# CliMA/ClimaSeaIce.jl

Hardware: AMD Instinct MI355X
Metric: EVP sub-cycle cell-updates/s (higher is better)
Workload: dtype f64; 1 GPU; evp_subcycle_fplane_periodic_2048x2048_as_1x1_tiles_of_2048x2048_120substeps; substeps=120, mode=fast, halo=4, halo_exchange=none (one tile)

## Files before the change

climaseaice.jl_amd/_lib.py:

```python
import ctypes as C
import os

_HERE = os.path.dirname(os.path.abspath(__file__))
LIB_PATH = os.environ.get("CSI_HIP_LIBRARY", os.path.join(_HERE, "libcsi_hip.so"))

OK = 0
PERIODIC, BOUNDED, FULLY_CONNECTED, LEFT_CONNECTED, RIGHT_CONNECTED, RIGHT_FOLDED, LEFT_CONNECTED_RIGHT_FOLDED = 0, 1, 2, 3, 4, 5, 6
METRIC_UNIFORM, METRIC_PER_J, METRIC_FULL = 0, 1, 2
FIELD_IDS = ["U", "V", "H", "A", "S11", "S22", "S12", "UN", "VN", "P", "ALPHA", "DELTA", "ZETA_F", "ZETA_C",
             "GH", "GA", "HM", "AM", "UM", "VM", "TOP_U", "TOP_V", "BOT_U", "BOT_V", "MASS_FLUX",
             "HS", "GHS", "HSM", "MASS_FLUX_SNOW", "SNOWFALL_INTERCEPTED", "TU", "TUS", "FORCING_U", "FORCING_V", "GU", "GV"]
THERMO_FIELD_IDS = ["TOP_HEAT_FLUX", "BOTTOM_HEAT_FLUX", "SNOWFALL"]
F = {n: k for k, n in enumerate(FIELD_IDS + THERMO_FIELD_IDS)}
STRESS_NONE, STRESS_CONST, STRESS_FIELD, STRESS_SEMI_IMPLICIT = 0, 1, 2, 3
VEL_ZERO, VEL_CONST, VEL_FIELD = 0, 1, 2
STRESS_TOP, STRESS_BOTTOM = 0, 1
MODE_STRICT, MODE_FAST = 0, 1
PRESSURE_REPLACEMENT, PRESSURE_ICE_STRENGTH = 0, 1
RHEOLOGY_EVP, RHEOLOGY_VISCOUS = 0, 1
SOLVER_SPLIT_EXPLICIT, SOLVER_EXPLICIT = 0, 1
FLUX_CONSTANT, FLUX_ARRAY, FLUX_RADIATIVE_EMISSION = 0, 1, 2
HEAT_TOP, HEAT_BOTTOM = 0, 1
MAX_HEAT_FLUX_TERMS = 8

SYMBOLS = ["csi_version", "csi_context_create", "csi_context_destroy", "csi_last_error", "csi_sync", "csi_set_mode",
           "csi_grid_set", "csi_mask_set", "csi_field_bind", "csi_evp_params_set", "csi_stress_set",
           "csi_evp_initialize", "csi_evp_subcycle", "csi_evp_finalize", "csi_time_step_momentum",
           "csi_compute_tracer_tendencies", "csi_dynamic_step_tracers", "csi_cache_current_fields",
           "csi_update_state", "csi_fill_halo_local", "csi_time_step_fe", "csi_time_step_rk3",
           "csi_slab_thermo_step", "csi_slab_params_set", "csi_layered_thermo_step", "csi_snow_params_set", "csi_tile_set", "csi_comm_unique_id", "csi_comm_init", "csi_comm_count", "csi_local_group_create", "csi_local_group_destroy", "csi_comm_init_local", "csi_comm_init_host", "csi_halo_exchange",
           "csi_plan_exchange", "csi_set_fusion", "csi_set_exchange_interval", "csi_set_halo_transport", "csi_halo_transport", "csi_set_peer_tier", "csi_peer_tier", "csi_plan_ranges", "csi_profile_substeps", "csi_last_path", "csi_last_subcycle_ms", "csi_launches_per_substep", "csi_last_launches", "csi_plan_pair", "csi_plan_peer_chunks", "csi_free_drift_set", "csi_coriolis_rows_set", "csi_velocity_bc_set",
           "csi_immersed_flux_bc_set", "csi_coriolis_points_set", "csi_validate_all", "csi_debug_peer_abort", "csi_set_weno_weight_dtype", "csi_weno_weight_dtype", "csi_subcycle_stats_begin", "csi_subcycle_stats_end",
           "csi_set_tile_skipping", "csi_tile_activity", "csi_set_row_constant", "csi_row_constant_rows",
           "csi_rheology_set", "csi_momentum_solver_set", "csi_compute_momentum_tendencies",
           "csi_heat_fluxes_set", "csi_surface_solve_set"]


class Metrics(C.Structure):
    _fields_ = [("dx", C.c_double), ("dy", C.c_double),
                ("dxc", C.POINTER(C.c_double)), ("dxf", C.POINTER(C.c_double)),
                ("azc", C.POINTER(C.c_double)), ("azf", C.POINTER(C.c_double)),
                ("full", C.POINTER(C.c_double) * 12), ("full_ld", C.c_int64)]


class EvpParams(C.Structure):
    _fields_ = [("ice_compressive_strength", C.c_double), ("ice_compaction_hardening", C.c_double),
                ("yield_curve_eccentricity", C.c_double), ("minimum_plastic_stress", C.c_double),
                ("min_relaxation_parameter", C.c_double), ("max_relaxation_parameter", C.c_double),
# ... 74 lines not shown
        "csi_snow_params_set": [vp, C.POINTER(SnowParams)],
        "csi_tile_set": [vp, i32, i32, i32, i32, i32, i32],
        "csi_comm_unique_id": [C.POINTER(C.c_uint8)],
        "csi_comm_init": [vp, i32, i32, C.POINTER(C.c_uint8)],
        "csi_comm_count": [vp, C.POINTER(i32)],
        "csi_local_group_create": [i32, C.POINTER(vp)], "csi_comm_init_local": [vp, vp, i32],
        "csi_comm_init_host": [vp, C.c_char_p, i32, i32],
        "csi_halo_exchange": [vp, C.POINTER(i32), i32, i32],
        "csi_plan_ranges": [i32, i32, i32, i32, i32, i32, i32, C.POINTER(i32)],
        "csi_plan_pair": [i32, i32, i32, i32, i32, i32, i32, i32, C.POINTER(i32)],
        "csi_plan_peer_chunks": [i32, i32, i32, i32, i32, i32, i32, C.POINTER(i32), C.POINTER(i32), i32],
        "csi_set_exchange_interval": [vp, i32],
        "csi_set_halo_transport": [vp, i32], "csi_halo_transport": [vp, C.POINTER(i32)],
        "csi_set_peer_tier": [vp, i32], "csi_peer_tier": [vp, C.POINTER(i32)],
        "csi_set_fusion": [vp, i32], "csi_free_drift_set": [vp, i32],
        "csi_set_tile_skipping": [vp, i32], "csi_tile_activity": [vp, C.POINTER(i32), C.POINTER(i32), C.POINTER(i32)],
        "csi_set_row_constant": [vp, i32, dbl], "csi_row_constant_rows": [vp, C.POINTER(i32)],
        "csi_coriolis_rows_set": [vp, C.POINTER(C.c_double), C.POINTER(C.c_double), i32],
        "csi_velocity_bc_set": [vp, i32, i32, i32, dbl],
        "csi_coriolis_points_set": [vp, C.POINTER(C.c_double), C.POINTER(C.c_double), i64],
        "csi_immersed_flux_bc_set": [vp, i32, dbl, dbl, dbl, dbl],
        "csi_plan_exchange": [i32] * 14 + [C.POINTER(i32)],
        "csi_profile_substeps": [vp, dbl, i32, C.POINTER(dbl)],
        "csi_last_path": [vp, C.POINTER(i32), C.POINTER(i32), C.POINTER(i32)],
        "csi_last_subcycle_ms": [vp, C.POINTER(dbl)], "csi_launches_per_substep": [vp, C.POINTER(i32)],
        "csi_last_launches": [vp, C.POINTER(i32), C.POINTER(i32)],
        "csi_validate_all": [vp], "csi_debug_peer_abort": [vp], "csi_set_weno_weight_dtype": [vp, i32], "csi_weno_weight_dtype": [vp, C.POINTER(i32)], "csi_subcycle_stats_begin": [vp],
        "csi_subcycle_stats_end": [vp, C.POINTER(dbl), C.POINTER(i32), C.POINTER(i32)],
        "csi_rheology_set": [vp, i32, dbl], "csi_momentum_solver_set": [vp, i32], "csi_compute_momentum_tendencies": [vp, dbl],
        "csi_heat_fluxes_set": [vp, i32, C.POINTER(HeatFluxTerm), i32], "csi_surface_solve_set": [vp, C.POINTER(SurfaceSolve)],
# ... 22 lines not shown


def plan_pair(Nx, Ny, Hx, Hy, topo_x, topo_y, k=1, m=0):
    L = load()
    out = (C.c_int32 * 32)()
    rc = L.csi_plan_pair(Nx, Ny, Hx, Hy, topo_x, topo_y, k, m, out)
    if rc != OK:
        raise CsiError(rc, "csi_plan_pair")
    if not out[0]:
        return None
    r = lambda q: tuple(out[4 + 4 * q: 8 + 4 * q])
    return dict(nstrips=out[1], nchunks=out[2], rows=out[3], first_compute=r(0), second_compute=r(1), store_sigma=r(2),
                store_first_u=r(3), store_first_v=r(4), store_second=r(5), walls=bool(out[28]))


def plan_peer_chunks(Nx, Ny, Hx, Hy, peer_south=True, peer_north=True):
    out = (C.c_int32 * 8)()
    rows = (C.c_int32 * 4096)()
    rc = load().csi_plan_peer_chunks(Nx, Ny, Hx, Hy, int(peer_south), int(peer_north), 256, out, rows, 2048)
    if rc != OK:
        raise CsiError(rc, "csi_plan_peer_chunks")
    if not out[0]:
        return None
    n = out[2]
    return dict(nstrips=out[1], nchunks=n, rows=out[3], elo=out[4], ehi=out[5], nS=out[6], nN=out[7],
                chunks=[(rows[2 * q], rows[2 * q + 1]) for q in range(min(n, 2048))])


def plan_exchange(Nx, Ny, Hx, Hy, topo_x, topo_y, rx, ry, Rx, Ry, periodic_x, periodic_y, width, halo):
    out = (C.c_int32 * 40)()
# ... 101 lines not shown
```

climaseaice.jl_amd/csrc/csi_abi.hip:

```cpp
#include "csi_ctx.h"


static SlabDev slab_dev(const csi_slab_params* p) {
    SlabDev S{};
    S.k = p->conductivity; S.rho_bulk = p->sea_ice_density; S.rho_pure = p->density; S.rho_l = p->liquid_density;
    S.c_l = p->liquid_heat_capacity; S.c_i = p->heat_capacity; S.L0 = p->reference_latent_heat; S.T0 = p->reference_temperature;
    S.liq_slope = p->liquidus_slope; S.liq_T0 = p->freshwater_melting_temperature; S.S = p->bottom_salinity;
    S.hc = p->ice_consolidation_thickness; S.Tu = p->top_temperature; S.Qu = p->top_heat_flux; S.Qb = p->bottom_heat_flux;
    S.top_flux_kind = p->top_flux_kind; S.bot_flux_kind = p->bottom_flux_kind;
    S.top_bc_kind = p->top_bc_kind; S.ice_salinity = p->ice_salinity;
    return S;
}
static SnowDev snow_dev(const csi_snow_params* p) {
    SnowDev W{};
    W.k = p->conductivity; W.rho = p->snow_density; W.snowfall = p->snowfall; W.Tu = p->top_temperature; W.top_bc_kind = p->top_bc_kind;
    return W;
}
static bool flux_path(const csi_context* c, bool snow) {
    const HeatFluxDev& F = c->heat;
    return F.top.n > 0 || F.bot.n > 0 || F.prescribed_array || (snow && F.snowfall_array);
}
static bool has_array_term(const FluxTermsDev& t) {
    for (int k = 0; k < t.n; ++k)
        if (t.kind[k] == FLUX_ARRAY) return true;
// ... 94 lines not shown
        auto env_int = [](const char* name) { const char* e = getenv(name); return (e && *e) ? atoi(e) : -1; };
        c->tune.fused_rows = env_int("CSI_FUSED_ROWS"); c->tune.pair_tiles = env_int("CSI_PAIR_TILES");
        c->tune.pair_minrows = env_int("CSI_PAIR_MINROWS"); c->tune.pair_rows = env_int("CSI_PAIR_ROWS");
        c->tune.pair_common = env_int("CSI_PAIR_COMMON"); c->tune.no_geom_sig = env_int("CSI_DEBUG_NO_GEOM_SIG");
        c->tune.peer_edge = env_int("CSI_PEER_EDGE");
        c->tune.write_through = env_int("CSI_WRITE_THROUGH");
        c->tune.adv_nt = env_int("CSI_ADV_NT"); c->tune.pair_target = env_int("CSI_PAIR_TARGET");
        { const char* e = getenv("CSI_ADV_STAGE_MAX_CELLS"); if (e && *e) c->tune.adv_stage_max_cells = atol(e); }
        { const int v = env_int("CSI_ROW_TARGET_1024"); if (v >= 0) c->tune.row_target_1024 = v; }
        { const int v = env_int("CSI_TILE_SKIPPING"); if (v >= 0) c->act.enabled = v != 0; }
        { const int v = env_int("CSI_ROW_CONSTANT"); if (v >= 0) c->rc_enabled = v != 0; }
        c->tune.band_fused = env_int("CSI_BAND_FUSED"); c->tune.band_event_flags = env_int("CSI_BAND_EVENT_FLAGS");
        c->tune.band_cus = env_int("CSI_BAND_CUS"); c->tune.band_cus_share = env_int("CSI_BAND_CUS_SHARE");
        c->tune.exp_band_only = env_int("CSI_EXP_BAND_ONLY");
        c->tune.exp_overlap = env_int("CSI_EXP_OVERLAP");
        c->tune.peer_kernel = env_int("CSI_PEER_KERNEL");
    }
    *out = c;
    return CSI_OK;
}

int32_t csi_context_destroy(csi_context* c) {
    if (!c) return CSI_OK;
    hipSetDevice(c->device);
    hipStreamSynchronize(c->stream);
    if (c->dev_metrics) hipFree(c->dev_metrics);
    if (c->dev_fcor) hipFree(c->dev_fcor);
    if (c->dev_fcor2) hipFree(c->dev_fcor2);
    peer_release(c);
    if (c->peer.slots) hipFree(c->peer.slots);
// ... 71 lines not shown

int32_t csi_set_mode(csi_context* c, int32_t mode) {
    if (!c) return CSI_ERR_INVALID_ARGUMENT;
    if (mode != CSI_MODE_STRICT && mode != CSI_MODE_FAST) return fail(c, CSI_ERR_INVALID_ARGUMENT, "unknown mode");
    c->mode = mode;
    return CSI_OK;
}

int32_t csi_set_tile_skipping(csi_context* c, int32_t on) {
    if (!c) return CSI_ERR_INVALID_ARGUMENT;
    c->act.enabled = on ? 1 : 0;
    c->act.scale = 1.0; c->act.last_live = -1; c->act.last_tiles = 0; c->act.last_used = 0; c->act.since_probe = 0;
    return CSI_OK;
}

int32_t csi_tile_activity(csi_context* c, int32_t* tiles, int32_t* live, int32_t* used) {
    if (!c) return CSI_ERR_INVALID_ARGUMENT;
    activity_sample(c);
    if (tiles) *tiles = c->act.last_tiles;
    if (live) *live = c->act.last_live;
    if (used) *used = c->act.last_used;
    return CSI_OK;
}

int32_t csi_set_row_constant(csi_context* c, int32_t on, double rtol) {
    if (!c) return CSI_ERR_INVALID_ARGUMENT;
    if (!(rtol >= 0.0) || rtol > 1e-6) return fail(c, CSI_ERR_INVALID_ARGUMENT, "row-constant tolerance: 0 <= rtol <= 1e-6");
    c->rc_enabled = on ? 1 : 0;
    c->rc_rtol = rtol;
    c->rc_dirty = true;
// ... 666 lines not shown
    memset(out32, 0, 32 * sizeof(int32_t));
    out32[0] = (pair_supported(&tmp) && (!tiled || k % 2 == 0)) ? 1 : 0;
    if (!out32[0]) return CSI_OK;
    const int W = 2 * k;
    const SideV va = pair_side_v(&tmp, W - 2 * m, 4), vb = pair_side_v(&tmp, W - 2 * m - 2, 2);
    const Range ra = v_stress_range(&tmp, va), dec = v_stress_range(&tmp, vb);
    const FusedGeom G = pair_geom(&tmp, dec);
    out32[1] = G.nstrips; out32[2] = G.nchunks; out32[3] = G.rows;
    const Range r[6] = {ra, dec, clip_store(&tmp, dec, true), clip_store(&tmp, v_first_range(&tmp, vb, true), false),
                        clip_store(&tmp, v_first_range(&tmp, vb, false), false), clip_store(&tmp, v_second_range(&tmp, vb), false)};
    for (int q = 0; q < 6; ++q) { out32[4 + 4 * q] = r[q].i0; out32[5 + 4 * q] = r[q].i1; out32[6 + 4 * q] = r[q].j0; out32[7 + 4 * q] = r[q].j1; }
    out32[28] = has_walls(&tmp) ? 1 : 0;
    return CSI_OK;
}

int32_t csi_plan_peer_chunks(int32_t Nx, int32_t Ny, int32_t Hx, int32_t Hy, int32_t peer_south, int32_t peer_north, int32_t cus,
                             int32_t* out8, int32_t* rows_out, int32_t max_chunks) {
    if (!out8 || !rows_out || Nx < 1 || Ny < 1 || max_chunks < 1) return CSI_ERR_INVALID_ARGUMENT;
    csi_context tmp;
    tmp.Nx = Nx; tmp.Ny = Ny; tmp.Hx = Hx; tmp.Hy = Hy;
    tmp.g.xlo = tmp.g.xhi = tmp.g.ylo = tmp.g.yhi = SIDE_PERIODIC;
    tmp.coef.uniform = 1; tmp.metric_kind = CSI_METRIC_UNIFORM;
    tmp.geom_peer = 1;
    for (int d = 0; d < 8; ++d) tmp.peer.sync_rank[d] = -1;
    if (peer_south) tmp.peer.sync_rank[2] = 0;
    if (peer_north) tmp.peer.sync_rank[3] = 0;
    (void)cus;
    memset(out8, 0, 8 * sizeof(int32_t));
    if (!pair_supported(&tmp)) return CSI_OK;
    const Range dec = v_stress_range(&tmp, pair_side_v(&tmp, 2, 2));
// ... 118 lines not shown
```

climaseaice.jl_amd/csrc/csi_core.hip:

```cpp
#include "csi_ctx.h"

namespace csi_host {

std::string g_create_error;


int32_t fail(csi_context* c, int32_t code, const std::string& msg) {
    if (c) c->err = msg; else g_create_error = msg;
    return code;
}

int side_lo(int topo) {
    switch (topo) {
        case CSI_PERIODIC: return SIDE_PERIODIC;
        case CSI_BOUNDED: return SIDE_WALL;
        case CSI_FULLY_CONNECTED: return SIDE_CONNECTED;
        case CSI_LEFT_CONNECTED: return SIDE_CONNECTED;
        case CSI_LEFT_CONNECTED_RIGHT_FOLDED: return SIDE_CONNECTED;
        default: return SIDE_WALL;
    }
}
int side_hi(int topo) {
    switch (topo) {
        case CSI_PERIODIC: return SIDE_PERIODIC;
// ... 364 lines not shown
    if (max_chunks < 1) max_chunks = 1;
    int rows = (height + max_chunks - 1) / max_chunks;
    if (!forced && rows < 16) {
        max_chunks = 1024 / G.nstrips;
        if (max_chunks < 1) max_chunks = 1;
        rows = (height + max_chunks - 1) / max_chunks;
    }
    int min_rows = 6;
    if (c->tune.pair_minrows >= 0) min_rows = c->tune.pair_minrows;
    if (rows < min_rows) rows = min_rows;
    if (c->tune.pair_rows >= 0) rows = c->tune.pair_rows;
    if (rows > height) rows = height;
    if (rows < 1) rows = 1;
    G.rows = rows;
    G.nchunks = (height + rows - 1) / rows;
    G.wt = c->tune.write_through >= 0 ? (c->tune.write_through != 0) : ((long)width * height <= kWriteThroughCells);
    if (c->geom_peer && !forced && c->tune.pair_rows < 0 && c->tune.peer_edge != 0) {
        for (;; ++rows) {
            const int reach = std::max(c->Hy, 4), want = rows - (c->tune.peer_edge > 0 ? c->tune.peer_edge : 4);
            const int e_lo = std::max(reach + 1 - dec.j0, want), e_hi = std::max(reach + (dec.j1 - c->Ny), want);
            const bool lo = c->peer.sync_rank[2] >= 0 && e_lo < rows, hi = c->peer.sync_rank[3] >= 0 && e_hi < rows;
            G.rows = rows; G.elo = G.ehi = 0;
            G.nchunks = (height + rows - 1) / rows;
            if (height >= 4 * rows && (lo || hi)) {
                G.elo = lo ? e_lo : rows;
                G.ehi = hi ? e_hi : 0;
                const int mid = height - G.elo - G.ehi;
                G.nchunks = 1 + (mid + rows - 1) / rows + (hi ? 1 : 0);
                if (!hi) {
                    G.nchunks = 1 + (height - G.elo + rows - 1) / rows;
                }
            }
            if (G.nchunks <= max_chunks || rows >= height) break;
        }
    }
    return G;
}


}
```

climaseaice.jl_amd/csrc/csi_ctx.h:

```cpp
#pragma once
#include "../../include/csi.h"
#include "csi_dev.h"
#include "csi_kernels.h"
#include "momentum_dev.h"
#include "csi_hostgroup.h"
#include "csi_comm.h"
#include <rccl/rccl.h>
#include <cmath>
#include <cstdio>
#include <cstring>
#include <cstdlib>
#include <chrono>
#include <condition_variable>
#include <deque>
#include <mutex>
#include <string>
#include <vector>
#include <algorithm>
#include <initializer_list>

using namespace csi;

namespace csi_host {

// ... 159 lines not shown
        double sample_scale[kSamples] = {1, 1, 1, 1};
        unsigned seq = 0;
        int seen_id = -1;
        double scale = 1.0;
        int last_live = -1, last_tiles = 0;
        int last_used = 0;
        int since_probe = 0;
    } act;
    std::vector<double> coef2_host, fcor2_host;
    double* dev_c2row = nullptr;
    int* dev_rcsum = nullptr;
    bool rc_dirty = true;
    int rc_enabled = 1;
    double rc_rtol = 0.0;
    int rc_rows = 0;
    int geom_band = 0;
    int geom_peer = 0;
    struct Tuning { int fused_rows = -1, pair_tiles = -1, pair_target = -1, row_target_1024 = 0, pair_minrows = -1, pair_rows = -1, pair_common = -1, peer_kernel = -1, peer_edge = -1, write_through = -1,
                    adv_nt = -1,
                    band_fused = -1,
                    band_event_flags = -1,
                    band_cus = -1,
                    band_cus_share = -1,
                    exp_band_only = -1,
                    exp_overlap = -1,
                    no_geom_sig = -1;
      long adv_stage_max_cells = 1L << 40;
    } tune;
};

namespace csi_host {

#define HIP_TRY(c, expr)                                                                        \
    do {                                                                                        \
        hipError_t e_ = (expr);                                                                 \
        if (e_ != hipSuccess)                                                                   \
            return fail(c, CSI_ERR_HIP, std::string(#expr) + ": " + hipGetErrorString(e_));     \
    } while (0)

#define NCCL_TRY(c, expr)                                                                       \
    do {                                                                                        \
        ncclResult_t r_ = (expr);                                                               \
        if (r_ != ncclSuccess)                                                                  \
            return fail(c, CSI_ERR_COMM, std::string(#expr) + ": " + ncclGetErrorString(r_));   \
    } while (0)

static inline int nxf_of(int k) { return k > 1 ? 5 : 2; }

struct FoldBand;
static const int kPing[5] = {CSI_F_U, CSI_F_V, CSI_F_S11, CSI_F_S22, CSI_F_S12};
struct FusedGeom { Range rs; int nstrips, nchunks, rows; int elo = 0, ehi = 0; int wt = 0; };
static inline void chunk_rows(const FusedGeom& G, int q, int* ja, int* jb) {
    const int elo = G.elo > 0 ? G.elo : G.rows;
    const bool last_short = G.ehi > 0 && q == G.nchunks - 1 && q > 0;
    *ja = last_short ? G.rs.j1 - G.ehi + 1 : G.rs.j0 + (q == 0 ? 0 : elo + (q - 1) * G.rows);
    *jb = q == 0 ? std::min(*ja + elo - 1, G.rs.j1) : (q == G.nchunks - 1 ? G.rs.j1 : std::min(*ja + G.rows - 1, G.rs.j1 - G.ehi));
}
constexpr int kMaxExchangeInterval = 16;
struct SideV { int xlo, xhi, ylo, yhi; };
static const int kPeerDx[8] = {-1, 1, 0, 0, -1, 1, -1, 1}, kPeerDy[8] = {0, 0, -1, 1, -1, -1, 1, 1};
static const int kPeerOpp[8] = {1, 0, 3, 2, 7, 6, 5, 4};
struct PeerSets { int nW, nE, nS, nN, size[8], n[8]; };
struct PeerRec {
    hipIpcMemHandle_t handle;
    uint64_t offset;
    int64_t ld;
    int32_t ok, pad;
    uint64_t local_ptr;
    int32_t set_size[8];
};
constexpr int kPeerRecs = csi_context::Peer::NARR + 1;
struct PeerView {
    csi_context* c; GridDev g; int Ny;
// ... 50 lines not shown
int32_t copy_parent(csi_context* c, int dst, int src);
int32_t do_initialize(csi_context* c);
FRef alt_ref(const csi_context* c, int k);
FusedGeom fused_geom(const csi_context* c, int V);
void velocity_ranges(const csi_context* c, bool ufirst, int V, Range& r1, Range& r1c, Range& r2);
int32_t ensure_alt(csi_context* c);
int exchange_interval(const csi_context* c);
SideV pair_side_v(const csi_context* c, int v_connected, int v_periodic);
Range v_first_range(const csi_context* c, const SideV& v, bool ufirst);
Range clip_store(const csi_context* c, Range r, bool sigma);
bool has_walls(const csi_context* c);
bool offsets_fit_32bit(int Nx, int Ny, int Hx, int Hy, int64_t max_ld);
int64_t max_bound_ld(const csi_context* c);
bool pair_supported(const csi_context* c);
FusedGeom pair_geom(const csi_context* c, const Range& dec, double tile_scale = 1.0);
int32_t ensure_row_constant(csi_context* c);
bool activity_sample(csi_context* c);
PeerSets peer_wait_counts(const csi_context* c, const FusedGeom& G);
void peer_local_arrays(const csi_context* c, const void* out[csi_context::Peer::NARR]);
void peer_release(csi_context* c);
bool fold_cut_possible(const csi_context* c);
bool peer_tile_supported(csi_context* c, const EvpDev& Pfull);
PeerSets peer_my_sets(csi_context* c);
int32_t peer_setup(csi_context* c, bool local_ok);
int32_t peer_decide(csi_context* c, const EvpDev& P, int substeps, bool* use);
int32_t peer_fill_table(csi_context* c, const FusedGeom& G, bool out_is_alt, FusedTable* t);
FRef band_ref(const csi_context* c, int q);
int32_t ensure_band(csi_context* c);
int32_t band_substep(csi_context* c, const FoldBand& bd, const FastCoef& fc, const FRef* b, const FRef* d, bool ufirst, int jlo, bool last, hipStream_t st);
int32_t band_substeps(csi_context* c, const FoldBand& bd, const FastCoef& fc, int cur, int s, int n, bool last);
// ... 32 lines not shown
```

climaseaice.jl_amd/csrc/csi_launch.hip:

```cpp
#include "csi_ctx.h"

namespace csi_host {

static int32_t stats_mark(csi_context* c) {
    if (!c->stats.on || c->stats.ev.size() >= 2 * 4096) return CSI_OK;
    hipEvent_t e;
    HIP_TRY(c, hipEventCreate(&e));
    HIP_TRY(c, hipEventRecord(e, c->stream));
    c->stats.ev.push_back(e);
    return CSI_OK;
}
static void stats_launches(csi_context* c, int n) { if (c->stats.on && c->stats.launches.size() * 2 < c->stats.ev.size()) c->stats.launches.push_back(n); }

bool activity_sample(csi_context* c) {
    csi_context::Activity& a = c->act;
    if (!a.host) return false;
    volatile int* w = a.host;
    const int s1 = w[0];
    if (s1 & 1) return false;
    __atomic_thread_fence(__ATOMIC_ACQUIRE);
    const int live = w[1], tiles = w[2], id = w[3];
    __atomic_thread_fence(__ATOMIC_ACQUIRE);
    if (w[0] != s1 || s1 == 0 || id == a.seen_id) return false;
    a.seen_id = id; a.last_live = live; a.last_tiles = tiles;
// ... 75 lines not shown
            xd_v.p = c->xd[1] + (c->Hx - 1) + (int64_t)(c->Hy - 1) * src[1]->ld; xd_v.ld = (int)src[1]->ld;
            launch_immersed_div(P, xd_u, xd_v, c->stream);
        }
    }
    const int kb = tiled ? k : (pairs ? 2 : 1);
    FRef orig[5], alt[5];
    for (int q = 0; q < 5; ++q) { orig[q] = ref_of(c, kPing[q]); alt[q] = alt_ref(c, q); }
    if (tiled && (rc = exchange_tile(orig))) return rc;
    const bool every_cell_written = pairs && !tiled && !has_walls(c) && substeps % 2 == 0;
    const ImageSpec imu = image_spec(c, CSI_F_U), imv = image_spec(c, CSI_F_V);
    constexpr int KMAX = kMaxExchangeInterval, NSINGLE = KMAX * 4, NPAIR = (KMAX / 2) * 4;
    if (k > KMAX) return fail(c, CSI_ERR_UNSUPPORTED, "exchange interval too large for the fused path");
    if (!c->dev_tables) HIP_TRY(c, hipMalloc((void**)&c->dev_tables, (NSINGLE + NPAIR) * sizeof(FusedTable)));
    FusedGeom G[KMAX], GP[KMAX / 2];
    FusedGeom GA{};
    bool act_on = c->act.enabled != 0 && pairs && !tiled && substeps >= 8;
    if (act_on) {
        csi_context::Activity& a = c->act;
        if (!a.list) {
            HIP_TRY(c, hipMalloc((void**)&a.flags, sizeof(int) * kMaxActTiles));
            HIP_TRY(c, hipMalloc((void**)&a.list, sizeof(int) * (kMaxActTiles + 2)));
            HIP_TRY(c, hipMalloc((void**)&a.list0, sizeof(int) * (kMaxActTiles + 2)));
            HIP_TRY(c, hipHostMalloc((void**)&a.host, sizeof(int) * 4, hipHostMallocMapped));
            memset(a.host, 0, sizeof(int) * 4);
            HIP_TRY(c, hipHostGetDevicePointer((void**)&a.host_dev, a.host, 0));
        }
        double s_scale = 1.0;
        bool fresh = false;
        if (csi_host::activity_sample(c)) { s_scale = a.sample_scale[(unsigned)a.seen_id % csi_context::Activity::kSamples]; fresh = true; }
        if (fresh && a.last_tiles > 0) {
// ... 70 lines not shown
                        Range rs = clip_store(c, dec, true), r1 = clip_store(c, v_first_range(c, vb, buf), false),
                              r2 = clip_store(c, v_second_range(c, vb), false);
                        if (band) {
                            rs.j1 = std::min(rs.j1, c->Ny); r1.j1 = std::min(r1.j1, c->Ny); r2.j1 = std::min(r2.j1, c->Ny);
                        }
                        FusedTable* t = &host[NSINGLE + (mp * 2 + cur) * 2 + auf];
                        fused_fill_table(P, fc, cur == 0 ? orig : alt, cur == 0 ? alt : orig, rs, r1, r1, r2, imu, imv, t);
                        fused_fill_pair_extra(dec, ra.j0, ra.j1, ims11, ims22, ims12, t, GP[mp].elo, GP[mp].ehi, GP[mp].wt);
                        if (force) { fused_fill_forcing(P, ubar_v, vbar_u, t); if (wind) fused_fill_forcing_top(P, tbar_v, tbar_u, t); }
                        if (extra) fused_fill_extra(P, xd_u, xd_v, t);
                        if (peer && (rc = peer_fill_table(c, GP[mp], cur == 0, t))) return rc;
                        if (act_on) { t->P[FP_ACT_LIVE] = (unsigned long)c->act.list; t->P[FP_ACT_LIVE0] = (unsigned long)c->act.list0; }
                    }
            }
        }
        HIP_TRY(c, hipMemcpyAsync(c->dev_tables, host, sizeof(FusedTable) * (NSINGLE + NPAIR), hipMemcpyHostToDevice, c->stream));
        HIP_TRY(c, hipEventRecord(c->ring_ev[slot], c->stream));
        c->ring_used[slot] = true;
    }
    unsigned long long peer_dld_bit = 0ull;
    if (peer)
        for (int d = 0; d < 8; ++d) if (c->peer.dld[d][0] | c->peer.dld[d][1]) peer_dld_bit = 1ull << 63;
    c->act.last_used = 0;
    if (act_on) {
        ActivityArgs A{};
        A.h = ref_of(c, CSI_F_H); A.a = ref_of(c, CSI_F_A);
        A.s11 = orig[2]; A.s22 = orig[3]; A.s12 = orig[4]; A.u = orig[0]; A.v = orig[1];
        A.rho = P.rho;
        A.dec = GA.rs;
        A.nstrips = GA.nstrips; A.nchunks = GA.nchunks; A.rows = GA.rows; A.elo = GA.elo; A.ehi = GA.ehi;
// ... 38 lines not shown
    }
    const bool skip_pair = band && c->tune.exp_band_only > 0;
    int nflip = 0;
    auto launch_stream = [&]() { return ps != c->stream ? ps : ((two_streams && (nflip++ & 1)) ? c->band_stream : c->stream); };
    for (int s = first; s < end;) {
        const bool ufirst = (s % 2) == 0;
        if (pairs && end - s >= 2 && m + 1 < kb) {
            const int mp = m / 2;
            if (band) {
                HIP_TRY(c, hipStreamWaitEvent(ps, c->band_ev_band, 0));
                if ((rc = band_substeps(c, *band, fc, cur, s, 2, s + 2 == end))) return rc;
                nlaunch += band_launches(c, 2);
            }
            const bool live_only = act_on && npair >= 2 && s + 2 != end;
            const bool start_only = q0_on && npair < 2 && s + 2 != end;
            const FusedGeom& GL = (live_only || start_only) ? GA : GP[mp];
            if (!skip_pair)
            launch_fused_pair(c->dev_tables + NSINGLE + ((mp * 2 + cur) * 2 + (ufirst ? 1 : 0)),
                              c->metric_kind == CSI_METRIC_FULL ? 2 : (c->coef.uniform != 0 ? 0 : 1), ufirst,
                              has_walls(c) || masked || force || peer_dld_bit != 0, masked, force, P.free_drift != 0, extra_kind, common_forcing, GL.nstrips, GL.nchunks, GL.rows,
                              (s + 2 == end ? 1 : 0) | (live_only ? 4 : 0) | (start_only ? 8 : 0),
                              peer ? (++c->peer.seq | peer_dld_bit) : (c->tune.peer_kernel > 0 ? 1ull : 0ull), launch_stream());
            ++npair;
            if (band) HIP_TRY(c, hipEventRecord(c->band_ev_pair, ps));
            m += 2; s += 2;
        } else if (single_by_pair) {
            if (band) {
                HIP_TRY(c, hipStreamWaitEvent(ps, c->band_ev_band, 0));
                if ((rc = band_substeps(c, *band, fc, cur, s, 1, s + 1 == end))) return rc;
                nlaunch += band_launches(c, 1);
            }
            if (!skip_pair)
            launch_fused_pair(c->dev_tables + ((m * 2 + cur) * 2 + (ufirst ? 1 : 0)),
// ... 40 lines not shown
    }
    HIP_TRY(c, hipEventRecord(c->ev1, c->stream));
    if ((rc = stats_mark(c))) return rc;
    stats_launches(c, nlaunch);
    if (cur == 1)
        for (int q = 0; q < 5; ++q) {
            const Bound& b = c->f[kPing[q]];
            HIP_TRY(c, hipMemcpyAsync(b.p, c->alt[q], c->alt_elems[q] * sizeof(double), hipMemcpyDeviceToDevice, c->stream));
        }
    HIP_TRY(c, hipGetLastError());
    c->last_exchanges = nex;
    c->last_k = k;
    c->last_launches = nlaunch;
    c->last_substeps = substeps;
    c->last_used_pairs = pairs && substeps >= 2;
    return CSI_OK;
}


int32_t run_fused_peer(csi_context* c, double dt, const FastCoef& fc, int substeps, int first) {
    int32_t rc;
    FRef orig[5];
    for (int q = 0; q < 5; ++q) orig[q] = ref_of(c, kPing[q]);
    if ((rc = ensure_alt(c))) return rc;
    const bool fold = c->g.yhi == SIDE_FOLD;
    if (has_walls(c) || fold)
        for (int q = 0; q < 5; ++q)
            HIP_TRY(c, hipMemcpyAsync(c->alt[q], c->f[kPing[q]].p, c->alt_elems[q] * sizeof(double), hipMemcpyDeviceToDevice, c->stream));
    const int W = std::min(std::min(c->Hx, c->Hy), 4);
    if ((rc = exchange_refs(c, orig, 5, W))) return rc;
// ... 73 lines not shown
        c->last_fused = 2;
        return CSI_OK;
    }
    const bool fuse = peer || (fast && c->fusion && substeps > 0 &&
                               (pair_only ? (pfk >= 0 && pair_supported(c) && (!tiled || k % 2 == 0) && substeps >= 2)
                                          : fused_supported(P)));
    if (fuse) {
        c->peer.last = peer ? 1 : 0;
        if ((rc = peer ? run_fused_peer(c, dt, fc, substeps, first) : run_fused(c, P, fc, substeps, first))) return rc;
        c->timed = true;
        c->launches_per_substep = 1 + ((tiled && k == 1) ? 3 : 0);
        c->last_fused = c->last_used_pairs ? 2 : 1;
        return CSI_OK;
    }
    c->last_fused = 0;
    c->peer.last = 0;
    if (tiled && (rc = exchange(c, uvs, nxf, W))) return rc;
    HIP_TRY(c, hipEventRecord(c->ev0, c->stream));
    if ((rc = stats_mark(c))) return rc;
    int m = 0, nex = 0;
    for (int s = first; s < first + substeps; ++s) {
        const int V = W - 2 * m;
        const Range rs = stress_range(c, V), ru1 = first_u_range(c, V), rv1 = first_v_range(c, V), r2 = second_range(c, V);
        if (fast) {
            P.write_diag = (s == first + substeps - 1);
            launch_fast_stress(P, rs, fc, c->stream);
        } else {
            launch_strict_visc(P, rs, c->stream);
            launch_strict_stress(P, rs, c->stream);
        }
// ... 166 lines not shown
```

climaseaice.jl_amd/model.py:

```python
import ctypes as C
from types import SimpleNamespace

import numpy as np
import torch

from . import _lib
from .dynamics import (ElastoViscoPlasticRheology, ExplicitSolver, FPlane, IceStrength, SeaIceMomentumEquation, SemiImplicitStress,
                       ViscousRheology)
from .fields import CenterField, Field, XFaceField, YFaceField
from .grids import (METRIC_NAMES, Bounded, Center, FullyConnected, LeftConnected, LeftConnectedRightFolded, Periodic, RightConnected,
                    RightFolded, TileGrid)


_OWN = object()


def _cell_shape_ok(value, grid):
    if isinstance(value, Field):
        return value.location == (Center, Center) and (value.ni, value.nj) == tuple(grid.field_size(Center, Center))
    shape = np.shape(value)
    if isinstance(grid, TileGrid) and shape == (grid.global_grid.Ny, grid.global_grid.Nx):
        return True
    return shape == (grid.Ny, grid.Nx)

# ... 508 lines not shown

    def external_stress_field(self, slot, comp):
        return self._stress_fields[f"{slot}_{comp}"]

    def set_mode(self, mode):
        self.mode = mode
        self.ctx.call("csi_set_mode", _lib.MODE_FAST if mode == "fast" else _lib.MODE_STRICT)

    def set_fusion(self, level):
        level = 2 if level is True else int(level)
        self.ctx.call("csi_set_fusion", level)

    def set_tile_skipping(self, on):
        self.ctx.call("csi_set_tile_skipping", 1 if on else 0)

    def tile_activity(self):
        import ctypes as C
        t, l, u = C.c_int32(0), C.c_int32(0), C.c_int32(0)
        self.ctx.call("csi_tile_activity", C.byref(t), C.byref(l), C.byref(u))
        return t.value, l.value, u.value

    def set_row_constant(self, on=True, rtol=0.0):
        self.ctx.call("csi_set_row_constant", 1 if on else 0, float(rtol))

    def row_constant_rows(self):
        import ctypes as C
        n = C.c_int32(0)
        self.ctx.call("csi_row_constant_rows", C.byref(n))
        return n.value

# ... 134 lines not shown
```

include/csi.h:

```cpp
#ifndef CSI_H
#define CSI_H

#include <stdint.h>

#ifdef __cplusplus
extern "C" {
#endif

#define CSI_VERSION 100

typedef enum {
    CSI_OK = 0,
    CSI_ERR_INVALID_ARGUMENT = -1,
    CSI_ERR_NOT_BOUND = -2,
    CSI_ERR_HIP = -3,
    CSI_ERR_UNSUPPORTED = -4,
    CSI_ERR_NO_DEVICE = -5,
    CSI_ERR_COMM = -6
} csi_status;

typedef enum {
    CSI_PERIODIC = 0,
    CSI_BOUNDED = 1,
    CSI_FULLY_CONNECTED = 2,
// ... 209 lines not shown
int32_t csi_halo_exchange(csi_context* ctx, const int32_t* field_ids, int32_t nfields, int32_t width);

int32_t csi_free_drift_set(csi_context* ctx, int32_t kind);

typedef enum { CSI_RHEOLOGY_EVP = 0, CSI_RHEOLOGY_VISCOUS = 1 } csi_rheology_kind;
typedef enum { CSI_SOLVER_SPLIT_EXPLICIT = 0, CSI_SOLVER_EXPLICIT = 1 } csi_momentum_solver_kind;
int32_t csi_rheology_set(csi_context* ctx, int32_t kind, double nu);
int32_t csi_momentum_solver_set(csi_context* ctx, int32_t kind);
int32_t csi_compute_momentum_tendencies(csi_context* ctx, double dt);

int32_t csi_set_fusion(csi_context* ctx, int32_t level);

int32_t csi_set_tile_skipping(csi_context* ctx, int32_t on);
int32_t csi_tile_activity(csi_context* ctx, int32_t* tiles, int32_t* live, int32_t* used);

int32_t csi_set_row_constant(csi_context* ctx, int32_t on, double rtol);
int32_t csi_row_constant_rows(csi_context* ctx, int32_t* rows);

int32_t csi_set_exchange_interval(csi_context* ctx, int32_t k);

enum { CSI_TRANSPORT_RCCL = 0, CSI_TRANSPORT_PEER = 1 };
int32_t csi_set_halo_transport(csi_context* ctx, int32_t kind);
int32_t csi_halo_transport(csi_context* ctx, int32_t* kind);
int32_t csi_set_peer_tier(csi_context* ctx, int32_t tier);
int32_t csi_peer_tier(csi_context* ctx, int32_t* tier);

int32_t csi_plan_ranges(int32_t Nx, int32_t Ny, int32_t Hx, int32_t Hy, int32_t topo_x, int32_t topo_y,
                        int32_t valid_width, int32_t* out16);

int32_t csi_plan_exchange(int32_t Nx, int32_t Ny, int32_t Hx, int32_t Hy, int32_t topo_x, int32_t topo_y,
                          int32_t rank_x, int32_t rank_y, int32_t Rx, int32_t Ry, int32_t periodic_x, int32_t periodic_y,
                          int32_t width, int32_t halo, int32_t* out40);

int32_t csi_last_subcycle_ms(csi_context* ctx, double* ms);
int32_t csi_subcycle_stats_begin(csi_context* ctx);
int32_t csi_subcycle_stats_end(csi_context* ctx, double* total_ms, int32_t* cycles, int32_t* launches);
int32_t csi_plan_pair(int32_t Nx, int32_t Ny, int32_t Hx, int32_t Hy, int32_t topo_x, int32_t topo_y, int32_t k, int32_t m,
                      int32_t* out32);
int32_t csi_plan_peer_chunks(int32_t Nx, int32_t Ny, int32_t Hx, int32_t Hy, int32_t peer_south, int32_t peer_north, int32_t cus,
                             int32_t* out8, int32_t* rows_out, int32_t max_chunks);

int32_t csi_profile_substeps(csi_context* ctx, double dt, int32_t substeps, double* out_ms4);
int32_t csi_last_path(csi_context* ctx, int32_t* fused, int32_t* exchange_interval, int32_t* exchanges);
int32_t csi_last_launches(csi_context* ctx, int32_t* launches, int32_t* substeps);
int32_t csi_launches_per_substep(csi_context* ctx, int32_t* n);

#ifdef __cplusplus
}
#endif
#endif
```

Before: 71.83 billion cell-updates/s.

## Rotate fused pair-kernel chunk boundaries across substep pairs for cache reuse

Adds a pair-rotation planner that builds several phase-shifted chunk geometries for the fused two-substep kernel. Successive pairs cycle through these geometries, and the first chunk's height is offset each time. It is enabled automatically when the working-set footprint is between about 1.2x and 3.2x of a 256 MB Infinity Cache estimate, for uniform unmasked wall-free cases. The intent is to shift where chunk seams fall so that the rows re-read across pairs hit the last-level cache more often. In exchange it may raise rows per chunk and adds one chunk per launch, plus extra table copies.

Result: no change. 72.06 billion cell-updates/s, median of 6 (+0.3%).

```diff
diff --git a/climaseaice.jl_amd/_lib.py b/climaseaice.jl_amd/_lib.py
--- a/climaseaice.jl_amd/_lib.py
+++ b/climaseaice.jl_amd/_lib.py
@@ -31,7 +31,7 @@
            "csi_slab_thermo_step", "csi_slab_params_set", "csi_layered_thermo_step", "csi_snow_params_set", "csi_tile_set", "csi_comm_unique_id", "csi_comm_init", "csi_comm_count", "csi_local_group_create", "csi_local_group_destroy", "csi_comm_init_local", "csi_comm_init_host", "csi_halo_exchange",
            "csi_plan_exchange", "csi_set_fusion", "csi_set_exchange_interval", "csi_set_halo_transport", "csi_halo_transport", "csi_set_peer_tier", "csi_peer_tier", "csi_plan_ranges", "csi_profile_substeps", "csi_last_path", "csi_last_subcycle_ms", "csi_launches_per_substep", "csi_last_launches", "csi_plan_pair", "csi_plan_peer_chunks", "csi_free_drift_set", "csi_coriolis_rows_set", "csi_velocity_bc_set",
            "csi_immersed_flux_bc_set", "csi_coriolis_points_set", "csi_validate_all", "csi_debug_peer_abort", "csi_set_weno_weight_dtype", "csi_weno_weight_dtype", "csi_subcycle_stats_begin", "csi_subcycle_stats_end",
-           "csi_set_tile_skipping", "csi_tile_activity", "csi_set_row_constant", "csi_row_constant_rows",
+           "csi_set_tile_skipping", "csi_tile_activity", "csi_set_pair_rotation", "csi_last_pair_rotation", "csi_plan_pair_rotation", "csi_set_row_constant", "csi_row_constant_rows",
            "csi_rheology_set", "csi_momentum_solver_set", "csi_compute_momentum_tendencies",
            "csi_heat_fluxes_set", "csi_surface_solve_set"]
 
@@ -136,6 +136,8 @@
         "csi_set_halo_transport": [vp, i32], "csi_halo_transport": [vp, C.POINTER(i32)],
         "csi_set_peer_tier": [vp, i32], "csi_peer_tier": [vp, C.POINTER(i32)],
         "csi_set_fusion": [vp, i32], "csi_free_drift_set": [vp, i32],
+        "csi_set_pair_rotation": [vp, i32], "csi_last_pair_rotation": [vp, C.POINTER(i32)],
+        "csi_plan_pair_rotation": [i32, i32, i32, i32, i32, i32, i32, dbl, C.POINTER(i32), C.POINTER(i32), i32],
         "csi_set_tile_skipping": [vp, i32], "csi_tile_activity": [vp, C.POINTER(i32), C.POINTER(i32), C.POINTER(i32)],
         "csi_set_row_constant": [vp, i32, dbl], "csi_row_constant_rows": [vp, C.POINTER(i32)],
         "csi_coriolis_rows_set": [vp, C.POINTER(C.c_double), C.POINTER(C.c_double), i32],
@@ -188,6 +190,21 @@
                 store_first_u=r(3), store_first_v=r(4), store_second=r(5), walls=bool(out[28]))
 
 
+def plan_pair_rotation(Nx, Ny, Hx, Hy, topo_x, topo_y, phases=0, f=0.0):
+    out = (C.c_int32 * 24)()
+    cap = 4096
+    rows = (C.c_int32 * (2 * 8 * cap))()
+    rc = load().csi_plan_pair_rotation(Nx, Ny, Hx, Hy, topo_x, topo_y, int(phases), float(f), out, rows, cap)
+    if rc != OK:
+        raise CsiError(rc, "csi_plan_pair_rotation")
+    if not out[0]:
+        return None
+    P = out[1]
+    return dict(phases=P, nstrips=out[2], rows=out[3], max_chunks=out[4], j0=out[5], j1=out[6],
+                nchunks=[out[8 + 2 * p] for p in range(P)], elo=[out[9 + 2 * p] for p in range(P)],
+                chunks=[[(rows[2 * (p * cap + q)], rows[2 * (p * cap + q) + 1]) for q in range(min(out[8 + 2 * p], cap))] for p in range(P)])
+
+
 def plan_peer_chunks(Nx, Ny, Hx, Hy, peer_south=True, peer_north=True):
     out = (C.c_int32 * 8)()
     rows = (C.c_int32 * 4096)()
diff --git a/climaseaice.jl_amd/csrc/csi_abi.hip b/climaseaice.jl_amd/csrc/csi_abi.hip
--- a/climaseaice.jl_amd/csrc/csi_abi.hip
+++ b/climaseaice.jl_amd/csrc/csi_abi.hip
@@ -132,6 +132,7 @@
         c->tune.band_cus = env_int("CSI_BAND_CUS"); c->tune.band_cus_share = env_int("CSI_BAND_CUS_SHARE");
         c->tune.exp_band_only = env_int("CSI_EXP_BAND_ONLY");
         c->tune.exp_overlap = env_int("CSI_EXP_OVERLAP");
+        { const char* e = getenv("CSI_PAIR_PHASE"); int P = 0; double f = 0.0; if (e && sscanf(e, "%d:%lf", &P, &f) == 2) { c->tune.pair_phases = P; c->tune.pair_phase_f = f; } }
         c->tune.peer_kernel = env_int("CSI_PEER_KERNEL");
     }
     *out = c;
@@ -233,6 +234,19 @@
     return CSI_OK;
 }
 
+int32_t csi_set_pair_rotation(csi_context* c, int32_t mode) {
+    if (!c) return CSI_ERR_INVALID_ARGUMENT;
+    if (mode != 0 && mode != 1) return fail(c, CSI_ERR_INVALID_ARGUMENT, "pair rotation: 0 (off) or 1 (auto)");
+    c->pair_rotation = mode;
+    return CSI_OK;
+}
+
+int32_t csi_last_pair_rotation(csi_context* c, int32_t* phases) {
+    if (!c || !phases) return CSI_ERR_INVALID_ARGUMENT;
+    *phases = c->last_pair_phases;
+    return CSI_OK;
+}
+
 int32_t csi_tile_activity(csi_context* c, int32_t* tiles, int32_t* live, int32_t* used) {
     if (!c) return CSI_ERR_INVALID_ARGUMENT;
     activity_sample(c);
@@ -929,6 +943,31 @@
     return CSI_OK;
 }
 
+int32_t csi_plan_pair_rotation(int32_t Nx, int32_t Ny, int32_t Hx, int32_t Hy, int32_t topo_x, int32_t topo_y, int32_t phases, double f,
+                               int32_t* out24, int32_t* rows_out, int32_t max_chunks) {
+    if (!out24 || !rows_out || Nx < 1 || Ny < 1 || max_chunks < 1 || phases < 0) return CSI_ERR_INVALID_ARGUMENT;
+    csi_context tmp;
+    tmp.Nx = Nx; tmp.Ny = Ny; tmp.Hx = Hx; tmp.Hy = Hy;
+    tmp.g.xlo = side_lo(topo_x); tmp.g.xhi = side_hi(topo_x); tmp.g.ylo = side_lo(topo_y); tmp.g.yhi = side_hi(topo_y);
+    tmp.coef.uniform = 1; tmp.metric_kind = CSI_METRIC_UNIFORM;
+    memset(out24, 0, 24 * sizeof(int32_t));
+    if (is_tiled(&tmp) || !pair_supported(&tmp)) return CSI_OK;
+    const Range dec = v_stress_range(&tmp, pair_side_v(&tmp, 2, 2));
+    const FusedGeom G0 = pair_geom(&tmp, dec);
+    const PairRotation R = pair_rotation_plan(&tmp, G0, phases, f);
+    out24[0] = 1; out24[1] = R.P; out24[2] = R.G[0].nstrips; out24[3] = R.G[0].rows; out24[4] = G0.max_chunks; out24[5] = dec.j0; out24[6] = dec.j1;
+    for (int p = 0; p < R.P; ++p) {
+        const FusedGeom& G = R.G[p];
+        out24[8 + 2 * p] = G.nchunks; out24[9 + 2 * p] = G.elo;
+        for (int q = 0; q < G.nchunks && q < max_chunks; ++q) {
+            int ja, jb;
+            chunk_rows(G, q, &ja, &jb);
+            rows_out[2 * (p * max_chunks + q)] = ja; rows_out[2 * (p * max_chunks + q) + 1] = jb;
+        }
+    }
+    return CSI_OK;
+}
+
 int32_t csi_plan_peer_chunks(int32_t Nx, int32_t Ny, int32_t Hx, int32_t Hy, int32_t peer_south, int32_t peer_north, int32_t cus,
                              int32_t* out8, int32_t* rows_out, int32_t max_chunks) {
     if (!out8 || !rows_out || Nx < 1 || Ny < 1 || max_chunks < 1) return CSI_ERR_INVALID_ARGUMENT;
diff --git a/climaseaice.jl_amd/csrc/csi_core.hip b/climaseaice.jl_amd/csrc/csi_core.hip
--- a/climaseaice.jl_amd/csrc/csi_core.hip
+++ b/climaseaice.jl_amd/csrc/csi_core.hip
@@ -402,6 +402,7 @@
     if (rows < 1) rows = 1;
     G.rows = rows;
     G.nchunks = (height + rows - 1) / rows;
+    G.max_chunks = max_chunks;
     G.wt = c->tune.write_through >= 0 ? (c->tune.write_through != 0) : ((long)width * height <= kWriteThroughCells);
     if (c->geom_peer && !forced && c->tune.pair_rows < 0 && c->tune.peer_edge != 0) {
         for (;; ++rows) {
@@ -425,5 +426,42 @@
     return G;
 }
 
-
-}
+constexpr double kInfinityCacheBytes = 256.0 * 1024.0 * 1024.0;
+constexpr double kPairRotationMinFootprint = 1.2, kPairRotationMaxFootprint = 3.2, kPairRotationFourPhases = 2.4;
+PairRotation pair_rotation_plan(const csi_context* c, const FusedGeom& G0, int phases, double f) {
+    PairRotation R;
+    R.G[0] = G0;
+    const int width = G0.rs.i1 - G0.rs.i0 + 1, height = G0.rs.j1 - G0.rs.j0 + 1;
+    if (phases == 0) {
+        if (c->tune.pair_phases >= 2) { phases = c->tune.pair_phases; f = c->tune.pair_phase_f; }
+        else {
+            const double fp = 15.0 * 8.0 * (double)width * (double)height / kInfinityCacheBytes;
+            const bool measured_family = c->coef.uniform != 0 && c->metric_kind != CSI_METRIC_FULL && !c->g.has_mask && !has_walls(c) &&
+                                         !evp_ring_forcing(evp_dev(c, 0.0));
+            if (!measured_family || !(fp > kPairRotationMinFootprint && fp <= kPairRotationMaxFootprint)) return R;
+            phases = fp > kPairRotationFourPhases ? 4 : 3;
+            f = 1.0 / phases;
+        }
+    }
+    if (phases < 2 || phases > kMaxPairPhases || !(f > 0.0 && f < 1.0)) return R;
+    if (G0.elo != 0 || G0.ehi != 0 || G0.max_chunks < 3 || G0.nchunks < 3) return R;
+    for (int rows = G0.rows; 2 * rows <= height; ++rows) {
+        bool fits = true;
+        for (int p = 0; p < phases && fits; ++p) {
+            int elo = (int)std::lround(std::fmod(p * (1.0 - f) * rows, (double)rows));
+            if (elo < 1 || elo > rows) elo = rows;
+            FusedGeom& G = R.G[p];
+            G = G0;
+            G.rows = rows;
+            G.elo = elo == rows ? 0 : elo;
+            G.nchunks = 1 + (height - elo + rows - 1) / rows;
+            fits = G.nchunks <= G0.max_chunks;
+        }
+        if (fits) { R.P = phases; return R; }
+    }
+    R.G[0] = G0;
+    return R;
+}
+
+
+}
diff --git a/climaseaice.jl_amd/csrc/csi_ctx.h b/climaseaice.jl_amd/csrc/csi_ctx.h
--- a/climaseaice.jl_amd/csrc/csi_ctx.h
+++ b/climaseaice.jl_amd/csrc/csi_ctx.h
@@ -197,9 +197,12 @@
     int rc_enabled = 1;
     double rc_rtol = 0.0;
     int rc_rows = 0;
+    int pair_rotation = 1;
+    int last_pair_phases = 1;
     int geom_band = 0;
     int geom_peer = 0;
     struct Tuning { int fused_rows = -1, pair_tiles = -1, pair_target = -1, row_target_1024 = 0, pair_minrows = -1, pair_rows = -1, pair_common = -1, peer_kernel = -1, peer_edge = -1, write_through = -1,
+                    pair_phases = -1,
                     adv_nt = -1,
                     band_fused = -1,
                     band_event_flags = -1,
@@ -208,6 +211,7 @@
                     exp_band_only = -1,
                     exp_overlap = -1,
                     no_geom_sig = -1;
+      double pair_phase_f = 0.0;
       long adv_stage_max_cells = 1L << 40;
     } tune;
 };
@@ -232,7 +236,7 @@
 
 struct FoldBand;
 static const int kPing[5] = {CSI_F_U, CSI_F_V, CSI_F_S11, CSI_F_S22, CSI_F_S12};
-struct FusedGeom { Range rs; int nstrips, nchunks, rows; int elo = 0, ehi = 0; int wt = 0; };
+struct FusedGeom { Range rs; int nstrips, nchunks, rows; int elo = 0, ehi = 0; int wt = 0; int max_chunks = 0; };
 static inline void chunk_rows(const FusedGeom& G, int q, int* ja, int* jb) {
     const int elo = G.elo > 0 ? G.elo : G.rows;
     const bool last_short = G.ehi > 0 && q == G.nchunks - 1 && q > 0;
@@ -240,6 +244,8 @@
     *jb = q == 0 ? std::min(*ja + elo - 1, G.rs.j1) : (q == G.nchunks - 1 ? G.rs.j1 : std::min(*ja + G.rows - 1, G.rs.j1 - G.ehi));
 }
 constexpr int kMaxExchangeInterval = 16;
+constexpr int kMaxPairPhases = kMaxExchangeInterval / 2;
+struct PairRotation { int P = 1; FusedGeom G[kMaxPairPhases]; };
 struct SideV { int xlo, xhi, ylo, yhi; };
 static const int kPeerDx[8] = {-1, 1, 0, 0, -1, 1, -1, 1}, kPeerDy[8] = {0, 0, -1, 1, -1, -1, 1, 1};
 static const int kPeerOpp[8] = {1, 0, 3, 2, 7, 6, 5, 4};
@@ -320,6 +326,7 @@
 int64_t max_bound_ld(const csi_context* c);
 bool pair_supported(const csi_context* c);
 FusedGeom pair_geom(const csi_context* c, const Range& dec, double tile_scale = 1.0);
+PairRotation pair_rotation_plan(const csi_context* c, const FusedGeom& G0, int phases = 0, double f = 0.0);
 int32_t ensure_row_constant(csi_context* c);
 bool activity_sample(csi_context* c);
 PeerSets peer_wait_counts(const csi_context* c, const FusedGeom& G);
diff --git a/climaseaice.jl_amd/csrc/csi_launch.hip b/climaseaice.jl_amd/csrc/csi_launch.hip
--- a/climaseaice.jl_amd/csrc/csi_launch.hip
+++ b/climaseaice.jl_amd/csrc/csi_launch.hip
@@ -113,6 +113,7 @@
     if (!c->dev_tables) HIP_TRY(c, hipMalloc((void**)&c->dev_tables, (NSINGLE + NPAIR) * sizeof(FusedTable)));
     FusedGeom G[KMAX], GP[KMAX / 2];
     FusedGeom GA{};
+    PairRotation ROT;
     bool act_on = c->act.enabled != 0 && pairs && !tiled && substeps >= 8;
     if (act_on) {
         csi_context::Activity& a = c->act;
@@ -213,6 +214,15 @@
                     }
             }
         }
+        if (pairs && c->pair_rotation != 0 && !tiled && !peer && !band && !act_on && substeps / 2 >= 3) {
+            ROT = pair_rotation_plan(c, GP[0]);
+            for (int p = 1; p < ROT.P; ++p)
+                for (int q = 0; q < 4; ++q) {
+                    FusedTable* t = &host[NSINGLE + p * 4 + q];
+                    *t = host[NSINGLE + q];
+                    t->I[FI_ELO] = ROT.G[p].elo;
+                }
+        }
         HIP_TRY(c, hipMemcpyAsync(c->dev_tables, host, sizeof(FusedTable) * (NSINGLE + NPAIR), hipMemcpyHostToDevice, c->stream));
         HIP_TRY(c, hipEventRecord(c->ring_ev[slot], c->stream));
         c->ring_used[slot] = true;
@@ -281,9 +291,10 @@
             }
             const bool live_only = act_on && npair >= 2 && s + 2 != end;
             const bool start_only = q0_on && npair < 2 && s + 2 != end;
-            const FusedGeom& GL = (live_only || start_only) ? GA : GP[mp];
+            const int ph = ROT.P > 1 ? npair % ROT.P : mp;
+            const FusedGeom& GL = (live_only || start_only) ? GA : (ROT.P > 1 ? ROT.G[ph] : GP[mp]);
             if (!skip_pair)
-            launch_fused_pair(c->dev_tables + NSINGLE + ((mp * 2 + cur) * 2 + (ufirst ? 1 : 0)),
+            launch_fused_pair(c->dev_tables + NSINGLE + ((ph * 2 + cur) * 2 + (ufirst ? 1 : 0)),
                               c->metric_kind == CSI_METRIC_FULL ? 2 : (c->coef.uniform != 0 ? 0 : 1), ufirst,
                               has_walls(c) || masked || force || peer_dld_bit != 0, masked, force, P.free_drift != 0, extra_kind, common_forcing, GL.nstrips, GL.nchunks, GL.rows,
                               (s + 2 == end ? 1 : 0) | (live_only ? 4 : 0) | (start_only ? 8 : 0),
@@ -354,6 +365,7 @@
     c->last_launches = nlaunch;
     c->last_substeps = substeps;
     c->last_used_pairs = pairs && substeps >= 2;
+    c->last_pair_phases = ROT.P;
     return CSI_OK;
 }
 
@@ -457,6 +469,7 @@
         return CSI_OK;
     }
     c->last_fused = 0;
+    c->last_pair_phases = 1;
     c->peer.last = 0;
     if (tiled && (rc = exchange(c, uvs, nxf, W))) return rc;
     HIP_TRY(c, hipEventRecord(c->ev0, c->stream));
diff --git a/climaseaice.jl_amd/model.py b/climaseaice.jl_amd/model.py
--- a/climaseaice.jl_amd/model.py
+++ b/climaseaice.jl_amd/model.py
@@ -546,6 +546,15 @@
     def set_tile_skipping(self, on):
         self.ctx.call("csi_set_tile_skipping", 1 if on else 0)
 
+    def set_pair_rotation(self, mode):
+        self.ctx.call("csi_set_pair_rotation", 1 if mode else 0)
+
+    def last_pair_rotation(self):
+        import ctypes as C
+        n = C.c_int32(1)
+        self.ctx.call("csi_last_pair_rotation", C.byref(n))
+        return n.value
+
     def tile_activity(self):
         import ctypes as C
         t, l, u = C.c_int32(0), C.c_int32(0), C.c_int32(0)
diff --git a/include/csi.h b/include/csi.h
--- a/include/csi.h
+++ b/include/csi.h
@@ -247,6 +247,9 @@
 int32_t csi_set_tile_skipping(csi_context* ctx, int32_t on);
 int32_t csi_tile_activity(csi_context* ctx, int32_t* tiles, int32_t* live, int32_t* used);
 
+int32_t csi_set_pair_rotation(csi_context* ctx, int32_t mode);
+int32_t csi_last_pair_rotation(csi_context* ctx, int32_t* phases);
+
 int32_t csi_set_row_constant(csi_context* ctx, int32_t on, double rtol);
 int32_t csi_row_constant_rows(csi_context* ctx, int32_t* rows);
 
@@ -273,6 +276,9 @@
 int32_t csi_plan_peer_chunks(int32_t Nx, int32_t Ny, int32_t Hx, int32_t Hy, int32_t peer_south, int32_t peer_north, int32_t cus,
                              int32_t* out8, int32_t* rows_out, int32_t max_chunks);
 
+int32_t csi_plan_pair_rotation(int32_t Nx, int32_t Ny, int32_t Hx, int32_t Hy, int32_t topo_x, int32_t topo_y, int32_t phases, double f,
+                               int32_t* out24, int32_t* rows_out, int32_t max_chunks);
+
 int32_t csi_profile_substeps(csi_context* ctx, double dt, int32_t substeps, double* out_ms4);
 int32_t csi_last_path(csi_context* ctx, int32_t* fused, int32_t* exchange_interval, int32_t* exchanges);
 int32_t csi_last_launches(csi_context* ctx, int32_t* launches, int32_t* substeps);
```
